# stripe/rainier

Hardware: AMD Instinct MI355X
Metric: leapfrog steps/sec (all chains) (higher is better)
Workload: dtype f64

## Files before the change

rainier_amd/csrc/engine.cpp:

```cpp
#include <hip/hip_runtime.h>
#include <hip/hiprtc.h>

#include <cmath>
#include <chrono>
#include <cstdio>
#include <cstdlib>
#include <cstring>
#include <algorithm>
#include <atomic>
#include <fstream>
#include <functional>
#include <map>
#include <memory>
#include <mutex>
#include <string>
#include <thread>
#include <vector>

#include <dlfcn.h>
#include <sys/stat.h>
#include <unistd.h>

#include "../../include/rainier_hip.h"
#include "../../include/rainier_hip_rir.h"
#include "device/rh_shared.h"
#include "rir.hpp"
#include "optimize.hpp"
#include "engine_internal.hpp"
#include "lanes_plan.hpp"

const char *const kSharedSrc =
#include "gen/rh_shared.inc"
    ;
const char *const kPreludeSrc =
#include "gen/rh_prelude.inc"
    ;
static const char *kEngineSrc =
#include "gen/rh_engine.inc"
    ;
namespace {
thread_local std::string g_err;
std::atomic<long> g_compiles{0};

uint64_t fnv1a(const std::string &s, uint64_t h = 1469598103934665603ULL) {
  for (unsigned char ch : s) { h ^= ch; h *= 1099511628211ULL; }
  return h;
}

std::string lib_dir() {
  Dl_info info;
  if (dladdr((void *)&fnv1a, &info) && info.dli_fname) {
    std::string p(info.dli_fname);
    auto pos = p.find_last_of('/');
// ... 71 lines not shown
  KSet variants[8];
  bool want_nuts = false;
  rh::Program prog;
  rh::EmitOptions eopt;
  rh::EmitInfo info;
  int mass_vec = 9;
  std::string source, err, arch;
  std::vector<char> code;
  int device = 0;
  bool loaded = false;
  hipModule_t module = nullptr;
  hipFunction_t k_chain = nullptr, k_density = nullptr, k_selftest = nullptr, k_grad = nullptr, k_tick = nullptr;
  hipFunction_t k_grad_fused = nullptr;
  hipFunction_t k_absorb = nullptr;
  hipFunction_t k_compact = nullptr;
  int ncols_max = 0, glm_ncols = 0;
  hipFunction_t k_grad_glm = nullptr;
  bool glm_small = false;
  bool lk_lds = false;
  bool has_glm = false;
  int n_row_targets_hint = 0;
  bool shape_guessed = false;
  bool rows_unroll_auto = true;
  bool unroll_auto = false;
  int gather_waves = 3;
  int glm_w = 4;
  int n_row_targets = 0, grad_k = 4, nacc_max = 1;
  hipFunction_t k_grad_gather = nullptr, k_density_fin = nullptr;
  hipFunction_t k_grad_gather_scan = nullptr;
  std::vector<std::vector<int>> goff_host;
// ... 48 lines not shown
  int chains = 0;
  void *d_state = nullptr, *d_seeds = nullptr, *d_mass = nullptr, *d_draws = nullptr, *d_stats = nullptr, *d_running = nullptr;
  int it_done = 0;
  bool started = false, warmed = false;
  hipEvent_t e0 = nullptr, e1 = nullptr;
  double kernel_ms = 0, total_ms = 0;
  int64_t chain_slots = 0, steady_launches = 0, steady_evals = 0;
  double steady_ms = 0;
  int64_t launches = 0;
  bool tick_engine = false;
  int nsplit = 0, xcd_aware = 1;
  bool compact = true;
  void *d_qbuf = nullptr, *d_active = nullptr;
  void *d_rec[2] = {nullptr, nullptr};
  bool fuse = false;
  std::vector<Lane> lanes;
  std::vector<rh_chain_stats_dev> last_stats;
  int64_t grads_at_reset = 0;
};
int guard(rh_model *m, const std::function<void()> &fn) {
  try { fn(); return RH_OK; }
  catch (const Fail &f) { g_err = f.msg; if (m) m->err = f.msg; return f.code; }
  catch (const std::exception &e) { g_err = e.what(); if (m) m->err = e.what(); return RH_E_INVALID; }
}
DrawsView sampler_draws(rh_sampler *s) {
  return {s->d_draws, s->m->device, s->m->stream, s->chains, s->it_done, (int)s->m->prog.n_params, s->cfg.iterations, &s->m->mu, &s->m->err, s->m};
}

namespace {

// ... 266 lines not shown
    if (bad("rh_chain_kernel") && m->eopt.chain_waves != 1 && !rh::knob("RH_CHAIN_WAVES")) { m->eopt.chain_waves = 1; again(); continue; }
    if (bad("rh_grad_kernel") || bad("rh_grad_fused_kernel")) {
      bool lighter = true;
      if (m->eopt.grad_unroll > 1) m->eopt.grad_unroll /= 2;
      else if (m->info.grad_k > 1) m->eopt.grad_chains = m->info.grad_k / 2;
      else if (m->eopt.grad_pipeline != 0) m->eopt.grad_pipeline = 0;
      else lighter = false;
      if (lighter) { again(); continue; }
    }
    if (!usable() && heavier()) { again(); continue; }
    if (marker) m->code = build_source(m->arch, m->source, extra);
    return;
  }
}

hipFunction_t fit_kernel(const std::vector<char> &code, hipModule_t module, const char *name, std::string *why = nullptr) {
  std::string w;
  const int h = kernel_health(code, name, &w);
  if (h != KH_OK) {
    if (why) *why = h == KH_BAD ? w : std::string(name) + " is not part of this build";
    return nullptr;
  }
  hipFunction_t f = nullptr;
  HIPCHK(hipModuleGetFunction(&f, module, name));
  return f;
}

void load_module(rh_model *m) {
  HIPCHK(hipSetDevice(m->device));
  HIPCHK(hipModuleLoadData(&m->module, m->code.data()));
  HIPCHK(hipModuleGetFunction(&m->k_selftest, m->module, "rh_selftest_kernel"));
// ... 130 lines not shown
  return ks;
}


int apply_compile_opts(rh_model *m, const rh_compile_opts *opts) {
  if (!opts) return -1;
  if (opts->struct_size != (int32_t)sizeof(rh_compile_opts)) throw Fail{RH_E_INVALID, "rh_compile_opts.struct_size mismatch"};
  if (opts->math_mode != RH_MATH_FAST && opts->math_mode != RH_MATH_STRICT) throw Fail{RH_E_INVALID, "unknown math_mode"};
  m->eopt.strict_math = opts->math_mode == RH_MATH_STRICT;
  m->eopt.fp_contract = opts->fp_contract != 0;
  if (opts->rows_unroll < 0 || opts->rows_unroll > 64) throw Fail{RH_E_INVALID, "rows_unroll out of range [0,64]"};
  if (opts->rows_unroll > 0) { m->eopt.rows_unroll = opts->rows_unroll; m->rows_unroll_auto = false; }
  if (opts->grad_chains < 0 || opts->grad_chains > 16 || opts->grad_unroll < 0 || opts->grad_unroll > 16)
    throw Fail{RH_E_INVALID, "grad_chains / grad_unroll out of range [0,16]"};
  m->eopt.grad_chains = opts->grad_chains; m->eopt.grad_unroll = opts->grad_unroll;
  m->eopt.factor_outputs = opts->factor_outputs != 0;
  if (opts->with_nuts < 0 || opts->with_nuts > 7) throw Fail{RH_E_INVALID, "with_nuts: unknown variant bits"};
  m->want_nuts = opts->with_nuts != 0;
  return opts->device;
}

void load_program(rh_model *m, const void *rir, size_t rir_len, const double *const *columns, const int64_t *nrows,
                  std::vector<const double *> &cols, std::vector<int64_t> &nrows_m, bool tables_without_data = false) {
  std::string err;
  if (!rh::parse_rir(rir, rir_len, m->prog, err)) throw Fail{RH_E_INVALID, err};
  if (m->prog.kind != 0) throw Fail{RH_E_INVALID, "a density program (header kind 0) is needed"};
  const uint32_t caller_cols = m->prog.n_cols_total;
  std::vector<uint32_t> old1, old2;
  bool lift = true;
  if (const char *e = rh::knob("RH_LIFT_CONSTANTS")) lift = std::atoi(e) != 0;
// ... 326 lines not shown
  const int rc = guard(m, [&] {
    int ndev = 0;
    if (hipGetDeviceCount(&ndev) != hipSuccess || ndev == 0) throw Fail{RH_E_DEVICE, "no HIP device available"};
    int dev = device;
    if (dev < 0) HIPCHK(hipGetDevice(&dev));
    if (dev >= ndev) throw Fail{RH_E_INVALID, "device ordinal out of range"};
    m->prog = src->prog; m->eopt = src->eopt; m->info = src->info; m->want_nuts = src->want_nuts;
    m->source = src->source; m->nacc_max = src->nacc_max; m->grad_k = src->grad_k; m->has_glm = src->has_glm;
    m->glm_small = src->glm_small; m->glm_w = src->glm_w; m->lk_lds = src->lk_lds; m->gather_waves = src->gather_waves;
    m->goff_host = src->goff_host; m->gather_count = src->gather_count; m->col_len = src->col_len; m->col_src = src->col_src;
    m->rows_total = src->rows_total; m->data = src->data; m->data.cols = nullptr;
    m->n_row_targets_hint = src->n_row_targets_hint; m->rows_unroll_auto = src->rows_unroll_auto; m->unroll_auto = src->unroll_auto;
    m->shape_guessed = src->shape_guessed; m->synth_cols = src->synth_cols; m->ncols_max = src->ncols_max; m->glm_ncols = src->glm_ncols;
    m->device = dev;
    m->arch = device_arch(dev);
    if (m->arch == src->arch) m->code = src->code; else build_code(m);
    load_module(m);
    if (m->want_nuts) (void)load_variant(m, 1);
    size_t c = 0;
    for (size_t t = 0; t < m->prog.targets.size(); t++) {
      const auto &T = m->prog.targets[t];
      for (uint32_t j = 0; j < T.n_cols; j++, c++) {
        const size_t bytes = (size_t)m->data.nrows[t] * sizeof(double);
        void *d = nullptr;
        HIPCHK(hipMalloc(&d, bytes ? bytes : 8));
        m->dev_cols.push_back(d);
        if (bytes) HIPCHK(hipMemcpyPeer(d, dev, src->dev_cols[c], src->device, bytes));
      }
    }
    for (size_t rt = 0; rt < src->goff_dev.size(); rt++) {
      const size_t bytes = m->goff_host[rt].size() * sizeof(int);
// ... 11 lines not shown
  *out = m;
  return RH_OK;
}

extern "C" void rh_model_destroy(rh_model *m) {
  if (!m) return;
  if (m->module || !m->dev_cols.empty()) {
    hipSetDevice(m->device);
    for (void *d : m->dev_cols) hipFree(d);
    if (m->d_coltab) hipFree(m->d_coltab);
    if (m->d_kpool) hipFree(m->d_kpool);
    for (void *d : m->goff_dev) hipFree(d);
    if (m->stream) hipStreamDestroy(m->stream);
    for (int v = 1; v < 8; v++)
      if (m->variants[v].module && m->variants[v].module != m->module) hipModuleUnload(m->variants[v].module);
    if (m->module) hipModuleUnload(m->module);
  }
  delete m;
}
extern "C" int rh_model_nvars(const rh_model *m) { return m ? (int)m->prog.n_params : -RH_E_INVALID; }
extern "C" const char *rh_model_hip_source(const rh_model *m) { return m ? m->source.c_str() : ""; }
extern "C" int rh_optimize(rh_model *m, const double *x0, int32_t starts, int32_t max_evals, double *x_out,
                           int32_t *evals_out, int32_t *status_out) {
  if (!m || !m->loaded) { g_err = "rh_optimize: model not loaded"; return RH_E_INVALID; }
  if (!x_out || starts <= 0) { m->err = g_err = "rh_optimize: bad arguments"; return RH_E_INVALID; }
  std::string err;
  int rc = rh::lbfgs_multistart((int)m->prog.n_params, starts, x0, max_evals,
                                [m](const double *q, int k, double *lp, double *gr) { return rh_density_eval(m, q, k, lp, gr); },
                                x_out, evals_out, status_out, err);
  (void)err;
// ... 70 lines not shown
extern "C" int rh_lower_report_data(const void *rir, size_t rir_len, const double *const *columns, const int64_t *nrows,
                                    const rh_compile_opts *opts, const char *arch, char **src_out, size_t *code_size, char **report) {
  rh_model m;
  const int rc = guard(nullptr, [&] {
    std::vector<int64_t> nrows_in;
    std::vector<const double *> colv;
    (void)apply_compile_opts(&m, opts);
    load_program(&m, rir, rir_len, columns, nrows, colv, nrows_in);
    bool all_cols = true;
    for (const double *c : colv) all_cols = all_cols && c != nullptr;
    if (all_cols && ((columns && nrows) || !m.synth_cols.empty())) { std::vector<int64_t> nrows_t; canonicalize(&m, colv.data(), nrows_in.data(), nrows_t); }
    assemble_source(&m);
    m.arch = arch && *arch ? arch : "gfx950";
    if (code_size) {
      build_code(&m);
      *code_size = m.code.size();
    }
    if (src_out) {
      std::string text = m.source;
      if (!m.info.kpool.empty()) {
        text += "\n// rh_kpool " + std::to_string(m.info.kpool.size()) + ":";
        char buf[40];
        for (double v : m.info.kpool) { std::snprintf(buf, sizeof buf, " %a", v); text += buf; }
        text += "\n";
      }
      *src_out = (char *)std::malloc(text.size() + 1); std::memcpy(*src_out, text.c_str(), text.size() + 1);
    }
    if (!code_size) return;
    std::vector<char> vcode;
    if (opts && opts->with_nuts) vcode = build_variant_code(&m, opts->with_nuts & 7);
    if (report) {
      std::string r = "attempts=" + std::to_string(m.compile_attempts) + " rows_unroll=" + std::to_string(m.eopt.rows_unroll) +
                      " grad_unroll=" + std::to_string(m.eopt.grad_unroll) + " grad_k=" + std::to_string(m.info.grad_k) +
                      " chain_waves=" + std::to_string(m.eopt.chain_waves) + " grad_pipeline=" + std::to_string(m.eopt.grad_pipeline) +
                      " chunk=" + std::to_string(m.eopt.chunk) + " bigu=" + std::to_string(m.eopt.big_unroll) + " gather=" + std::to_string((int)m.info.gather_mode) + " row_targets=" + std::to_string(m.n_row_targets_hint) + "\n";
      r += code_report(m.code, "base");
      if (!vcode.empty()) r += code_report(vcode, "variant" + std::to_string(opts->with_nuts & 7));
      *report = (char *)std::malloc(r.size() + 1); std::memcpy(*report, r.c_str(), r.size() + 1);
    }
  });
  return rc;
}
extern "C" int rh_lower_only(const void *rir, size_t rir_len, const rh_compile_opts *opts, const char *arch,
                             char **src_out, size_t *code_size) {
  return rh_lower_only_data(rir, rir_len, nullptr, nullptr, opts, arch, src_out, code_size);
}
extern "C" void rh_free(void *p) { std::free(p); }
extern "C" int rh_simplify_rir(const void *rir, size_t rir_len, int fast, void **out, size_t *out_len) {
  return guard(nullptr, [&] {
    rh::Program P; std::string err;
    if (!rh::parse_rir(rir, rir_len, P, err)) throw Fail{RH_E_INVALID, err};
    const std::vector<unsigned char> b = rh::write_rir(rh::simplify(P, fast != 0));
// ... 91 lines not shown
};

int default_nsplit(const rh_model *m, int chains) {
  const int ngroups = (chains + m->grad_k - 1) / m->grad_k;
  int64_t max_rows = 1;
  for (size_t t = 0; t < m->prog.targets.size(); t++) if (m->prog.targets[t].n_cols) max_rows = std::max<int64_t>(max_rows, m->data.nrows[t]);
  int nsplit = (int)std::max<int64_t>(1, ((m->eopt.grad_pipeline == 2 ? 2048 : 4096) + ngroups - 1) / ngroups);
  if (m->info.gather_mode) nsplit = (int)std::max<int64_t>(1, (16384 + ngroups - 1) / ngroups);
  if (const char *e = rh::knob("RH_GATHER_WG")) if (m->info.gather_mode) nsplit = (int)std::max<int64_t>(1, (std::atoi(e) + ngroups - 1) / ngroups);
  if (m->k_grad_glm) { const int ctiles = (chains + 15) / 16; nsplit = (int)std::max<int64_t>(1, (2048 + ctiles - 1) / ctiles); }
  nsplit = ((nsplit + 7) / 8) * 8;
  const int64_t cap = std::max<int64_t>(8, (max_rows / 2048) / 8 * 8);
  return (int)std::min<int64_t>(nsplit, cap);
}

void launch_grad(rh_model *m, GatherBufs *gb, void *d_q, void *d_list, void *d_nlive, void *d_vflag, void *d_partial, void *d_graderr, void *d_running,
                 int chains, int nsplit, int xcd, hipStream_t stream = nullptr) {
  if (!stream) stream = m->stream;
  const int ngroups = (chains + m->grad_k - 1) / m->grad_k;
  if (m->info.gather_mode) {
    void *ga[] = {&m->data, &gb->gd, &d_q, &d_list, &d_nlive, &d_vflag, &d_partial, &d_graderr, &d_running, &chains, &nsplit};
    if (gb->any_big) launch(m->k_grad_gather, (unsigned)(ngroups * nsplit), 64, stream, ga);
    if (gb->any_small) launch(m->k_grad_gather_scan, (unsigned)(ngroups * nsplit), 64, stream, ga);
    return;
  }
  void *args[] = {&m->data, &d_q, &d_list, &d_nlive, &d_vflag, &d_partial, &d_graderr, &d_running, &chains, &nsplit, &xcd};
  if (m->k_grad_glm) {
    const int ctiles = (chains + 15) / 16;
    const unsigned blocks = (unsigned)(((ctiles + m->glm_w - 1) / m->glm_w) * nsplit);
    const unsigned tile = (unsigned)m->glm_ncols * 66u * (unsigned)sizeof(double);
    const unsigned lds = (2u * tile + (m->lk_lds ? 6176u : 0u) <= 160u * 1024u ? 2u : 1u) * tile;
    HIPCHK(hipModuleLaunchKernel(m->k_grad_glm, blocks, 1, 1, 64u * m->glm_w, 1, 1, lds, stream, args, nullptr));
  } else
// ... 16 lines not shown
  if (use_tick && !m->tick_ok) { m->err = g_err = "the tick engine's kernels of this model are not fit to run: " + m->tick_why; return RH_E_UNSUPPORTED; }
  if (!use_tick && !m->density_ok) { m->err = g_err = "rh_density_kernel of this model is not fit to run: " + m->density_why; return RH_E_UNSUPPORTED; }
  std::lock_guard<std::mutex> lk(m->mu);
  int lookup_err = 0;
  const int rc = guard(m, [&] {
    HIPCHK(hipSetDevice(m->device));
    const int n = (int)m->prog.n_params;
    DevBuf bq(sizeof(double) * n * chains), bl(sizeof(double) * chains), bg(sizeof(double) * n * chains), be(sizeof(int));
    const bool bigth = m->info.bign && !m->info.gather_mode && (n > 512 || m->eopt.chunk > 0);
    DevBuf btot(bigth ? sizeof(double) * (size_t)(n + 1) * chains : 8);
    void *dq = bq.p, *dl = bl.p, *dg = bg.p, *de = be.p, *dtot = btot.p;
    HIPCHK(hipMemcpyAsync(dq, q, sizeof(double) * n * chains, hipMemcpyHostToDevice, m->stream));
    HIPCHK(hipMemsetAsync(de, 0, sizeof(int), m->stream));
    int ch = chains;
    if (use_tick) {
      int nsplit = grad_splits > 0 ? grad_splits : (m->info.gather_mode ? 64 : default_nsplit(m, chains));
      GatherBufs gb;
      if (m->info.gather_mode) gb.build(m, chains, nsplit);
      const size_t pbytes = sizeof(double) * (size_t)m->n_row_targets * nsplit * chains * m->nacc_max;
      DevBuf bpart(pbytes), brun(sizeof(int)), blist(sizeof(int) * chains);
      { std::vector<int> ident((size_t)chains);
        for (int c = 0; c < chains; c++) ident[(size_t)c] = c;
        HIPCHK(hipMemcpyAsync(blist.p, ident.data(), sizeof(int) * chains, hipMemcpyHostToDevice, m->stream));
        HIPCHK(hipStreamSynchronize(m->stream)); }
      HIPCHK(hipMemsetAsync(bpart.p, 0, pbytes, m->stream));
      int xcd = 1;
      if (const char *e = rh::knob("RH_XCD_AWARE")) xcd = std::atoi(e);
      void *dnl = nullptr;
      std::unique_ptr<DevBuf> bnl;
      if (const char *e = rh::knob("RH_EVAL_LIVE")) {
        std::vector<int> live;
        for (const char *p = e; *p;) { char *q2; long v = std::strtol(p, &q2, 10); if (q2 == p) break; if (v >= 0 && v < chains) live.push_back((int)v); p = *q2 ? q2 + 1 : q2; }
        std::sort(live.begin(), live.end());
        live.erase(std::unique(live.begin(), live.end()), live.end());
        if (!live.empty()) {
          const int nl = (int)live.size();
          HIPCHK(hipMemcpyAsync(blist.p, live.data(), sizeof(int) * nl, hipMemcpyHostToDevice, m->stream));
          bnl.reset(new DevBuf(sizeof(int)));
          HIPCHK(hipMemcpyAsync(bnl->p, &nl, sizeof(int), hipMemcpyHostToDevice, m->stream));
          HIPCHK(hipStreamSynchronize(m->stream));
          dnl = bnl->p;
        }
      }
      launch_grad(m, &gb, dq, blist.p, dnl, nullptr, bpart.p, de, brun.p, chains, nsplit, xcd);
      void *dpart = bpart.p;
      if (m->info.gather_mode) {
        void *fa[] = {&m->data, &gb.gd, &dq, &dpart, &dl, &dg, &de, &ch, &nsplit, &dtot};
        launch(m->k_density_fin, (unsigned)chains, 64, m->stream, fa);
      } else {
        void *fa[] = {&m->data, &dq, &dpart, &dl, &dg, &de, &ch, &nsplit, &dtot};
        launch(m->k_density_fin, (unsigned)chains, 64, m->stream, fa);
      }
      HIPCHK(hipMemcpyAsync(logp, dl, sizeof(double) * chains, hipMemcpyDeviceToHost, m->stream));
      HIPCHK(hipMemcpyAsync(grad, dg, sizeof(double) * n * chains, hipMemcpyDeviceToHost, m->stream));
      HIPCHK(hipMemcpyAsync(&lookup_err, de, sizeof(int), hipMemcpyDeviceToHost, m->stream));
      HIPCHK(hipStreamSynchronize(m->stream));
      return;
    }
    void *args[] = {&m->data, &dq, &dl, &dg, &de, &ch, &dtot};
// ... 168 lines not shown
      for (int c = 0; c < chains; c++) {
        const double nn = cfg->rng_next_gaussian ? cfg->rng_next_gaussian[c] : std::nan("");
        rec[2 * c] = seeds[c];
        std::memcpy(&rec[2 * c + 1], &nn, sizeof nn);
      }
      HIPCHK(hipMemcpy(s->d_seeds, rec.data(), sizeof(int64_t) * rec.size(), hipMemcpyHostToDevice));
    }
    std::vector<double> mass(n, 1.0);
    if (cfg->mass_tuner == RH_MASS_STATIC_DIAG) mass.assign(cfg->static_mass, cfg->static_mass + n);
    HIPCHK(hipMemcpy(s->d_mass, mass.data(), sizeof(double) * n, hipMemcpyHostToDevice));
    HIPCHK(hipMemset(s->d_draws, 0, draws_bytes));
    HIPCHK(hipEventCreate(&s->e0));
    HIPCHK(hipEventCreate(&s->e1));
    s->last_stats.resize(chains);
    if (s->tick_engine) {
      int nsplit = cfg->grad_splits;
      if (nsplit <= 0) nsplit = default_nsplit(m, chains);
      int subf = cfg->sampler == RH_SAMPLER_HMC ? 1 : 8;
      if (const char *e = rh::knob("RH_SUBF")) { subf = 1; while (subf * 2 <= std::atoi(e) && subf < 64) subf *= 2; }
      if (const char *e = rh::knob("RH_COMPACT")) s->compact = std::atoi(e) != 0;
      { int64_t max_rows = 1;
        for (size_t t = 0; t < m->prog.targets.size(); t++) if (m->prog.targets[t].n_cols) max_rows = std::max<int64_t>(max_rows, m->data.nrows[t]);
        while (subf > 1 && max_rows / ((int64_t)nsplit * subf) < 1024) subf >>= 1; }
      if (!m->k_compact) s->compact = false;
      nsplit *= subf;
      if (nsplit > 65536) throw Fail{RH_E_INVALID, "grad_splits too large"};
      s->nsplit = nsplit;
      if (const char *e = rh::knob("RH_XCD_AWARE")) s->xcd_aware = std::atoi(e);
      HIPCHK(hipMalloc(&s->d_qbuf, sizeof(double) * n * chains));
      HIPCHK(hipMalloc(&s->d_active, sizeof(int) * chains));
      HIPCHK(hipMemset(s->d_qbuf, 0, sizeof(double) * n * chains));
      HIPCHK(hipMemset(s->d_active, 0, sizeof(int) * chains));
      const size_t rec_u64 = (size_t)(3 * n + 8);
      {
        bool fuse = m->k_grad_fused && m->k_absorb && s->k_tick == m->k_tick && cfg->sampler == RH_SAMPLER_HMC && !m->k_grad_glm;
        if (const char *e = rh::knob("RH_FUSE")) fuse = fuse && std::atoi(e) != 0;
        if (fuse) {
          const size_t rec_bytes = sizeof(uint64_t) * rec_u64 * chains;
          for (int k = 0; k < 2; k++) { HIPCHK(hipMalloc(&s->d_rec[k], rec_bytes)); HIPCHK(hipMemset(s->d_rec[k], 0, rec_bytes)); }
          s->fuse = true;
        }
      }
      int forced = 0;
      if (const char *e = rh::knob("RH_LANES")) forced = std::atoi(e) == 1 ? 1 : (std::atoi(e) == 2 ? 2 : 0);
      const rh_plan::LaneCut cut = rh_plan::lanes_cut(chains, m->k_grad_glm ? 16 : m->grad_k, nsplit, m->k_grad_glm ? m->glm_w : 1,
                                                      device_cus(m->device), forced);
      s->lanes.resize((size_t)cut.lanes);
      const size_t iters_alloc = (size_t)cfg->iterations;
      for (int li = 0; li < cut.lanes; li++) {
        Lane &L = s->lanes[(size_t)li];
        const int f = cut.first[li], lc = cut.count[li];
        L.first = f; L.chains = lc;
        if (li == 0) L.stream = m->stream;
        else { HIPCHK(hipStreamCreateWithFlags(&L.stream, hipStreamNonBlocking)); L.own_stream = true; }
        HIPCHK(hipEventCreate(&L.e0));
        HIPCHK(hipEventCreate(&L.e1));
        L.state = (uint64_t *)s->d_state + (size_t)f * s->state_words;
        L.seeds = (int64_t *)s->d_seeds + (size_t)2 * f;
        L.draws = (double *)s->d_draws + (size_t)f * iters_alloc * n;
        L.stats = (rh_chain_stats_dev *)s->d_stats + f;
        L.qbuf = (double *)s->d_qbuf + (size_t)f * n;
// ... 64 lines not shown
                      &L.active, &partial, &L.d_graderr, &lst, &nl, &chains, &nsplit, &stop, &fresh};
      launch(s->k_tick, (unsigned)chains, 64, L.stream, args);
    } else {
      void *args[] = {&m->data, &s->cfg, &L.state, &L.seeds, &s->d_mass, &L.draws, &L.stats, &L.d_running, &L.qbuf,
                      &L.active, &partial, &L.d_graderr, &lst, &nl, &chains, &nsplit, &stop, &fresh};
      launch(s->k_tick, (unsigned)chains, 64, L.stream, args);
    }
    if (s->compact) {
      void *lg = (int *)L.d_livelog + log_slot;
      void *ca[] = {&L.active, &L.d_list, &L.d_nlive, &lg, &chains};
      launch(m->k_compact, 1u, 1024, L.stream, ca);
    }
  };
  auto grad = [&](Lane &L, void *partial) {
    launch_grad(m, L.gb, L.qbuf, L.d_list, s->compact ? L.d_nlive : nullptr ,
                value_free ? L.active : nullptr, partial, L.d_graderr, L.d_running, L.chains, nsplit, xcd, L.stream);
  };
  auto grad_fused = [&](Lane &L, void *partial_in, void *partial_out, void *rec_in, void *rec_out) {
    int chains = L.chains;
    void *live_n = s->compact ? L.d_nlive : nullptr;
    void *args[] = {&m->data, &L.qbuf, &L.d_list, &live_n, &partial_in, &partial_out, &L.d_graderr, &L.d_running, &L.state, &rec_in, &rec_out,
                    &chains, &nsplit, &xcd};
    launch(m->k_grad_fused, (unsigned)(((chains + m->grad_k - 1) / m->grad_k) * nsplit), 64, L.stream, args);
  };
  auto absorb = [&](Lane &L, void *rec) {
    int chains = L.chains;
    void *args[] = {&L.state, &rec, &L.qbuf, &L.active, &chains};
    launch(m->k_absorb, (unsigned)chains, 64, L.stream, args);
  };
  const int Ltraj = std::max(1, s->cfg.hmc_steps);
  const bool fuse_now = s->fuse && s->warmed && s->cfg.sampler == RH_SAMPLER_HMC && Ltraj > 1;
// ... 271 lines not shown
  if (warmed) *warmed = s->warmed ? 1 : 0;
  if (iterations_done) *iterations_done = s->it_done;
  return RH_OK;
}
extern "C" int rh_sampler_timing(rh_sampler *s, rh_timing *out, int reset) {
  if (!s || !out) { g_err = "rh_sampler_timing: NULL"; return RH_E_INVALID; }
  std::lock_guard<std::mutex> lk(s->m->mu);
  return guard(s->m, [&] {
    fetch_stats(s);
    int64_t grads = 0;
    for (auto &d : s->last_stats) grads += d.gradient_evaluations;
    std::memset(out, 0, sizeof(*out));
    out->kernel_ms = s->kernel_ms; out->total_ms = s->total_ms; out->launches = s->launches;
    out->density_evals = grads - s->grads_at_reset;
    out->row_chain_evals = out->density_evals * s->m->rows_total;
    std::snprintf(out->dominant_kernel, sizeof out->dominant_kernel, s->tick_engine ? (s->m->info.gather_mode ? "rh_grad_gather_kernel" : s->m->k_grad_glm ? "rh_grad_glm_kernel" : (s->fuse && s->warmed && s->cfg.hmc_steps > 1) ? "rh_grad_fused_kernel" : "rh_grad_kernel") : "rh_chain_kernel");
    out->chain_slots = s->tick_engine ? s->chain_slots : out->density_evals;
    out->steady_kernel_ms = s->steady_ms; out->steady_launches = s->steady_launches; out->steady_density_evals = s->steady_evals;
    if (reset) { s->kernel_ms = 0; s->total_ms = 0; s->launches = 0; s->grads_at_reset = grads; s->chain_slots = 0; s->steady_ms = 0; s->steady_launches = 0; s->steady_evals = 0; }
  });
}

extern "C" int rh_sample(rh_model *m, const rh_config *cfg, const int64_t *seeds, int32_t chains, double *draws,
                         double *mass_diag, rh_chain_stats *stats) {
  rh_sampler *s = nullptr;
  int rc = rh_sampler_create(m, cfg, seeds, chains, &s);
  if (rc != RH_OK) return rc;
  rc = rh_sampler_warmup(s);
  if (rc == RH_OK) rc = rh_sampler_run(s, cfg->iterations);
  if (rc == RH_OK && draws && cfg->iterations > 0) rc = rh_sampler_draws(s, 0, cfg->iterations, draws);
  if (rc == RH_OK) rc = rh_sampler_stats(s, stats, mass_diag);
  rh_sampler_destroy(s);
  return rc;
}

extern "C" int rh_sample_multi(rh_model *const *models, int32_t n_models, const rh_config *cfg, const int64_t *seeds,
                               int32_t chains, double *draws, double *mass_diag, rh_chain_stats *stats) {
  if (!models || n_models <= 0 || !cfg || !seeds || chains <= 0) { g_err = "rh_sample_multi: bad arguments"; return RH_E_INVALID; }
  if (cfg->struct_size != (int32_t)sizeof(rh_config)) { g_err = "rh_config.struct_size mismatch"; return RH_E_INVALID; }
  const int nv = models[0] ? rh_model_nvars(models[0]) : -1;
  for (int g = 0; g < n_models; g++) {
    if (!models[g] || !models[g]->loaded) { g_err = "rh_sample_multi: model " + std::to_string(g) + " not loaded"; return RH_E_INVALID; }
    if (rh_model_nvars(models[g]) != nv) { g_err = "rh_sample_multi: the models differ (nvars)"; return RH_E_INVALID; }
  }
  const int G = std::min<int>(n_models, chains);
  int splits_all = cfg->grad_splits;
  if (splits_all <= 0 && models[0]->n_row_targets > 0) splits_all = default_nsplit(models[0], chains);
  std::vector<int> first((size_t)G + 1, 0);
  for (int g = 0; g < G; g++) first[(size_t)g + 1] = first[(size_t)g] + chains / G + (g < chains % G ? 1 : 0);
  std::vector<int> rcs((size_t)G, RH_OK);
  std::vector<std::string> errs((size_t)G);
  std::vector<std::thread> th;
  for (int g = 0; g < G; g++)
    th.emplace_back([&, g] {
      const int c0 = first[(size_t)g], nc = first[(size_t)g + 1] - c0;
      rh_config c = *cfg;
      c.grad_splits = splits_all;
      if (cfg->rng_next_gaussian) c.rng_next_gaussian = cfg->rng_next_gaussian + c0;
      const size_t per_chain = (size_t)cfg->iterations * (size_t)nv;
      rcs[(size_t)g] = rh_sample(models[g], &c, seeds + c0, nc, draws ? draws + (size_t)c0 * per_chain : nullptr,
                                 mass_diag ? mass_diag + (size_t)c0 * nv : nullptr, stats ? stats + c0 : nullptr);
      if (rcs[(size_t)g] != RH_OK) errs[(size_t)g] = rh_last_error(models[g]);
    });
  for (auto &t : th) t.join();
  for (int g = 0; g < G; g++)
    if (rcs[(size_t)g] != RH_OK) { g_err = "shard " + std::to_string(g) + ": " + errs[(size_t)g]; return rcs[(size_t)g]; }
  return RH_OK;
}
```

rainier_amd/csrc/lanes_plan.hpp:

```cpp
#ifndef RH_LANES_PLAN_HPP
#define RH_LANES_PLAN_HPP

#include <algorithm>
#include <vector>

namespace rh_plan {
struct LaneCut { int lanes, first[2], count[2]; };
inline LaneCut lanes_cut(int chains, int group, int nsplit, int waves_per_wg, int cus, int forced) {
  LaneCut one = {1, {0, 0}, {chains, 0}};
  const int ngroups = (chains + group - 1) / group;
  if (forced == 1 || ngroups < 2) return one;
  const int cg = std::max(1, std::min(ngroups - 1, (chains + group) / (2 * group)));
  const int cut = cg * group;
  const long long smaller = std::min(cg, ngroups - cg);
  if (forced != 2 && smaller * nsplit * waves_per_wg < 4LL * cus) return one;
  return {2, {0, cut}, {cut, chains - cut}};
}

inline double busy_shares(int n, const double *t0, const double *t1, double *share) {
  struct End { double t; int kind, i; };
  std::vector<End> ends;
  ends.reserve((size_t)2 * n);
  for (int i = 0; i < n; i++) {
    share[i] = 0.0;
    ends.push_back({t0[i], 0, i});
    ends.push_back({std::max(t0[i], t1[i]), 1, i});
  }
  std::sort(ends.begin(), ends.end(), [](const End &a, const End &b) { return a.t != b.t ? a.t < b.t : (a.kind != b.kind ? a.kind < b.kind : a.i < b.i); });
  std::vector<int> open;
  double uni = 0.0, prev = 0.0;
  for (const End &e : ends) {
// ... 14 lines not shown
```

Before: 3.057 million.

## Add lane-walk gradient kernel with chain-per-lane row streaming for large HMC runs

Adds a separate gradient kernel in which each lane owns chains (two chains per lane) and the waves of a workgroup stream disjoint row ranges. Column values are read through the constant address space, R rows are unrolled at a time, and per-wave partial sums are reduced through shared memory. The kernel is compiled separately and only kept if it has no spills or scratch use. It is selected automatically for static HMC with many chains and many row evaluations, and comes with its own split count. Fused gradient kernels are turned off when it is selected, and the extra compile adds build time and code complexity.

```diff
diff --git a/rainier_amd/csrc/device/rh_lane.hip.h b/rainier_amd/csrc/device/rh_lane.hip.h
--- /dev/null
+++ b/rainier_amd/csrc/device/rh_lane.hip.h
@@ -0,0 +1,108 @@
+#if RH_NROWTARGETS > 0 && !RH_HAS_GATHER && !RH_BIGTH && !RH_BIGN && !RH_LK_LDS
+#ifndef RH_LANE_W
+#define RH_LANE_W 8
+#endif
+#ifndef RH_LANE_R
+#define RH_LANE_R 8
+#endif
+#ifndef RH_LANE_C
+#define RH_LANE_C 2
+#endif
+typedef const double __attribute__((address_space(4))) *rh_ccol_t;
+template <int T, bool NV>
+RH_DEV void rh_lane_targets(const double (&th)[RH_LANE_C][RH_NTH], const rh_model_data &d, const int w, const int split, const int nsplit,
+                            const int *__restrict__ lp, const int nvalid, const int chains, double *__restrict__ partial,
+                            double *red, int &err) {
+  if constexpr (T < RH_NTARGETS) {
+    typedef rh_target<T> TG;
+    if constexpr (TG::HAS_ROWS) {
+      constexpr int NC = TG::NCOLS, R = RH_LANE_R, C = RH_LANE_C, W = RH_LANE_W;
+      constexpr int NA = TG::NACC > 0 ? TG::NACC : 1;
+      const int lane = threadIdx.x & 63;
+      double inv[C][TG::NINV > 0 ? TG::NINV : 1];
+#pragma unroll
+      for (int k = 0; k < C; k++) TG::invariants(th[k], inv[k], err);
+      const long long n = d.nrows[T];
+      const long long blocks = (n + R - 1) / R, per = (blocks + nsplit - 1) / nsplit, perw = (per + W - 1) / W;
+      long long s0 = (long long)split * per * R, s1 = s0 + per * R;
+      if (s0 > n) s0 = n;
+      if (s1 > n) s1 = n;
+      long long r0 = s0 + (long long)w * perw * R, r1 = r0 + perw * R;
+      if (r0 > s1) r0 = s1;
+      if (r1 > s1) r1 = s1;
+      rh_ccol_t cp[NC];
+#pragma unroll
+      for (int j = 0; j < NC; j++) cp[j] = (rh_ccol_t)d.cols[TG::COL0 + j];
+      double acc[C][NA];
+#pragma unroll
+      for (int k = 0; k < C; k++)
+#pragma unroll
+        for (int o = 0; o < NA; o++) acc[k][o] = 0.0;
+      long long kb = r0;
+      for (; kb + R <= r1; kb += R) {
+        double c[R][NC];
+#pragma unroll
+        for (int u = 0; u < R; u++)
+#pragma unroll
+          for (int j = 0; j < NC; j++) c[u][j] = cp[j][kb + u];
+#pragma unroll
+        for (int u = 0; u < R; u++)
+#pragma unroll
+          for (int k = 0; k < C; k++) rh_row<TG, NV>(th[k], inv[k], c[u], acc[k], err);
+      }
+      for (; kb < r1; kb++) {
+        double c[NC];
+#pragma unroll
+        for (int j = 0; j < NC; j++) c[j] = cp[j][kb];
+#pragma unroll
+        for (int k = 0; k < C; k++) rh_row<TG, NV>(th[k], inv[k], c, acc[k], err);
+      }
+#pragma unroll
+      for (int k = 0; k < C; k++)
+#pragma unroll
+        for (int o = 0; o < NA; o++) red[((w * C + k) * NA + o) * 64 + lane] = acc[k][o];
+      __syncthreads();
+      for (int t = threadIdx.x; t < C * NA * 64; t += 64 * W) {
+        const int ko = t >> 6, l = t & 63, k = ko / NA, o = ko - k * NA;
+        double s = red[ko * 64 + l];
+#pragma unroll
+        for (int ww = 1; ww < W; ww++) s += red[(ww * C * NA + ko) * 64 + l];
+        const int slot = k * 64 + l;
+        if (slot < nvalid) partial[(((size_t)TG::ROWT * nsplit + split) * chains + lp[slot]) * RH_NACC_MAX + o] = s;
+      }
+      __syncthreads();
+    }
+    rh_lane_targets<T + 1, NV>(th, d, w, split, nsplit, lp, nvalid, chains, partial, red, err);
+  }
+}
+extern "C" __global__ void __launch_bounds__(64 * RH_LANE_W)
+rh_grad_lane_kernel(const rh_model_data d, const double *__restrict__ q, const int *__restrict__ list, const int *__restrict__ nlive,
+                    const int *__restrict__ vflag, double *__restrict__ partial, int *__restrict__ err_out, int *__restrict__ n_running,
+                    const int chains, const int nsplit, const int xcd_aware) {
+  __shared__ double red[RH_LANE_W * RH_LANE_C * RH_NACC_MAX * 64];
+  const int lane = threadIdx.x & 63, w = __builtin_amdgcn_readfirstlane((int)(threadIdx.x >> 6));
+  const int b = blockIdx.x;
+  if (b == 0 && threadIdx.x == 0) *n_running = 0;
+  const int nl = rh_live_count(nlive, chains);
+  int split, group;
+  rh_grad_map(b, nsplit, xcd_aware, split, group);
+  const int slot0 = group * (64 * RH_LANE_C);
+  if (slot0 >= nl) return;
+  double th[RH_LANE_C][RH_NTH];
+  bool gonly = rh_any_value_only<0>::v && vflag != nullptr;
+#pragma unroll
+  for (int k = 0; k < RH_LANE_C; k++) {
+    const int c = rh_live_chain(list, slot0 + k * 64 + lane, nl);
+    if constexpr (rh_any_value_only<0>::v) gonly = gonly && vflag[c] == 2;
+#pragma unroll
+    for (int i = 0; i < RH_NVARS; i++) th[k][i] = q[(size_t)c * RH_NVARS + i];
+  }
+  int err = 0;
+  if constexpr (rh_any_value_only<0>::v) {
+    if (__all(gonly)) rh_lane_targets<0, false>(th, d, w, split, nsplit, list + slot0, nl - slot0, chains, partial, red, err);
+    else rh_lane_targets<0, true>(th, d, w, split, nsplit, list + slot0, nl - slot0, chains, partial, red, err);
+  } else
+  rh_lane_targets<0, true>(th, d, w, split, nsplit, list + slot0, nl - slot0, chains, partial, red, err);
+  if (__any(err != 0) && lane == 0) atomicOr(err_out, 1);
+}
+#endif
diff --git a/rainier_amd/csrc/engine.cpp b/rainier_amd/csrc/engine.cpp
--- a/rainier_amd/csrc/engine.cpp
+++ b/rainier_amd/csrc/engine.cpp
@@ -13,6 +13,7 @@
 #include <map>
 #include <memory>
 #include <mutex>
+#include <sstream>
 #include <string>
 #include <thread>
 #include <vector>
@@ -37,6 +38,9 @@
     ;
 static const char *kEngineSrc =
 #include "gen/rh_engine.inc"
+    ;
+static const char *kLaneSrc =
+#include "gen/rh_lane.inc"
     ;
 namespace {
 thread_local std::string g_err;
@@ -138,6 +142,11 @@
   hipFunction_t k_grad_fused = nullptr;
   hipFunction_t k_absorb = nullptr;
   hipFunction_t k_compact = nullptr;
+  std::vector<char> lane_code;
+  hipModule_t lane_module = nullptr;
+  hipFunction_t k_grad_lane = nullptr;
+  int grad_chains_req = 0;
+  bool lane_tried = false;
   int ncols_max = 0, glm_ncols = 0;
   hipFunction_t k_grad_glm = nullptr;
   bool glm_small = false;
@@ -216,6 +225,7 @@
   void *d_qbuf = nullptr, *d_active = nullptr;
   void *d_rec[2] = {nullptr, nullptr};
   bool fuse = false;
+  bool lane_walk = false;
   std::vector<Lane> lanes;
   std::vector<rh_chain_stats_dev> last_stats;
   int64_t grads_at_reset = 0;
@@ -512,7 +522,64 @@
   }
 }
 
-hipFunction_t fit_kernel(const std::vector<char> &code, hipModule_t module, const char *name, std::string *why = nullptr) {
+int lane_ncols_max(const rh_model *m) {
+  int ncols_max = 0;
+  for (const auto &T : m->prog.targets) ncols_max = std::max<int>(ncols_max, (int)T.n_cols);
+  return ncols_max;
+}
+bool lane_eligible(const rh_model *m) {
+  const int ncols_max = lane_ncols_max(m);
+  const bool glm = m->has_glm && m->n_row_targets_hint == 1 && !m->glm_small;
+  return m->n_row_targets_hint > 0 && !m->info.gather_mode && !m->info.bign && m->eopt.chunk == 0 && !glm && !m->lk_lds &&
+         m->grad_chains_req == 0 && !m->want_nuts && rh_plan::lane_walk_fits_r(ncols_max, m->nacc_max, 4);
+}
+void build_lane_code(rh_model *m) {
+  m->lane_code.clear();
+  m->lane_tried = true;
+  if (!lane_eligible(m)) return;
+  const char *e = rh::knob("RH_HIPRTC_EXTRA");
+  const std::string extra = e ? e : "";
+  const bool cache = !std::getenv("RH_NO_KERNEL_CACHE");
+  for (int R : {8, 4}) {
+    if (!rh_plan::lane_walk_fits_r(lane_ncols_max(m), m->nacc_max, R)) continue;
+    const std::string src = (R == rh_plan::kLaneR ? std::string() : "#define RH_LANE_R " + std::to_string(R) + "\n") + m->source + "\n" + kLaneSrc;
+    const std::string marker = cache_path(m->arch, src, extra) + ".lane.unfit";
+    std::vector<char> mk;
+    if (cache && read_file(marker, mk) && std::string(mk.begin(), mk.end()).compare(0, marker_header().size(), marker_header()) == 0) continue;
+    bool fit = false;
+    std::string why;
+    rh::KernelMeta km;
+    std::vector<char> code;
+    try {
+      code = build_source(m->arch, src, extra, ".lane.co");
+      fit = kernel_health(code, "rh_grad_lane_kernel", &why) == KH_OK && rh::kernel_meta(code, "rh_grad_lane_kernel", km) && km.vgpr_spills == 0 &&
+            km.sgpr_spills == 0 && km.scratch_bytes == 0 && rh::kernel_touches_scratch(code, "rh_grad_lane_kernel") == 0;
+    } catch (const Fail &f) { why = f.msg; }
+    if (rh::knob("RH_BUILD_LOG"))
+      std::fprintf(stderr, "[rh build] lane walk R %d: vgprs %ld sgprs %ld spills %ld/%ld scratch %ld: %s %s\n", R, km.vgprs, km.sgprs, km.vgpr_spills,
+                   km.sgpr_spills, km.scratch_bytes, fit ? "fit" : "unfit", why.c_str());
+    if (fit) { m->lane_code = code; return; }
+    if (cache) {
+      std::remove((cache_path(m->arch, src, extra) + ".lane.co").c_str());
+      const std::string text = marker_header() + "\nrh_grad_lane_kernel\n";
+      write_file(marker, std::vector<char>(text.begin(), text.end()));
+    }
+  }
+}
+hipFunction_t fit_kernel(const std::vector<char> &code, hipModule_t module, const char *name, std::string *why = nullptr);
+hipFunction_t ensure_lane(rh_model *m) {
+  std::lock_guard<std::recursive_mutex> lk(m->engine_mu);
+  if (m->k_grad_lane) return m->k_grad_lane;
+  if (!m->k_grad || !m->k_tick || m->info.gather_mode) return nullptr;
+  if (!m->lane_tried) build_lane_code(m);
+  if (m->lane_code.empty() || m->lane_module) return nullptr;
+  HIPCHK(hipSetDevice(m->device));
+  HIPCHK(hipModuleLoadData(&m->lane_module, m->lane_code.data()));
+  m->k_grad_lane = fit_kernel(m->lane_code, m->lane_module, "rh_grad_lane_kernel", nullptr);
+  return m->k_grad_lane;
+}
+
+hipFunction_t fit_kernel(const std::vector<char> &code, hipModule_t module, const char *name, std::string *why) {
   std::string w;
   const int h = kernel_health(code, name, &w);
   if (h != KH_OK) {
@@ -673,6 +740,7 @@
   if (opts->grad_chains < 0 || opts->grad_chains > 16 || opts->grad_unroll < 0 || opts->grad_unroll > 16)
     throw Fail{RH_E_INVALID, "grad_chains / grad_unroll out of range [0,16]"};
   m->eopt.grad_chains = opts->grad_chains; m->eopt.grad_unroll = opts->grad_unroll;
+  m->grad_chains_req = opts->grad_chains;
   m->eopt.factor_outputs = opts->factor_outputs != 0;
   if (opts->with_nuts < 0 || opts->with_nuts > 7) throw Fail{RH_E_INVALID, "with_nuts: unknown variant bits"};
   m->want_nuts = opts->with_nuts != 0;
@@ -1029,7 +1097,9 @@
     m->shape_guessed = src->shape_guessed; m->synth_cols = src->synth_cols; m->ncols_max = src->ncols_max; m->glm_ncols = src->glm_ncols;
     m->device = dev;
     m->arch = device_arch(dev);
-    if (m->arch == src->arch) m->code = src->code; else build_code(m);
+    m->grad_chains_req = src->grad_chains_req;
+    if (m->arch == src->arch) { m->code = src->code; m->lane_code = src->lane_code; m->lane_tried = src->lane_tried; }
+    else build_code(m);
     load_module(m);
     if (m->want_nuts) (void)load_variant(m, 1);
     size_t c = 0;
@@ -1071,6 +1141,7 @@
     if (m->stream) hipStreamDestroy(m->stream);
     for (int v = 1; v < 8; v++)
       if (m->variants[v].module && m->variants[v].module != m->module) hipModuleUnload(m->variants[v].module);
+    if (m->lane_module) hipModuleUnload(m->lane_module);
     if (m->module) hipModuleUnload(m->module);
   }
   delete m;
@@ -1171,6 +1242,7 @@
     m.arch = arch && *arch ? arch : "gfx950";
     if (code_size) {
       build_code(&m);
+      build_lane_code(&m);
       *code_size = m.code.size();
     }
     if (src_out) {
@@ -1193,6 +1265,10 @@
                       " chunk=" + std::to_string(m.eopt.chunk) + " bigu=" + std::to_string(m.eopt.big_unroll) + " gather=" + std::to_string((int)m.info.gather_mode) + " row_targets=" + std::to_string(m.n_row_targets_hint) + "\n";
       r += code_report(m.code, "base");
       if (!vcode.empty()) r += code_report(vcode, "variant" + std::to_string(opts->with_nuts & 7));
+      if (!m.lane_code.empty()) {
+        std::istringstream all(code_report(m.lane_code, "lane"));
+        for (std::string ln; std::getline(all, ln);) if (ln.find("rh_grad_lane_kernel") != std::string::npos) r += ln + "\n";
+      }
       *report = (char *)std::malloc(r.size() + 1); std::memcpy(*report, r.c_str(), r.size() + 1);
     }
   });
@@ -1314,9 +1390,33 @@
   return (int)std::min<int64_t>(nsplit, cap);
 }
 
+int64_t lane_max_rows(const rh_model *m) {
+  int64_t max_rows = 1;
+  for (size_t t = 0; t < m->prog.targets.size(); t++) if (m->prog.targets[t].n_cols) max_rows = std::max<int64_t>(max_rows, m->data.nrows[t]);
+  return max_rows;
+}
+thread_local int g_total_chains = 0;
+thread_local int g_shard_walk = -1;
+bool walk_is_lane(rh_model *m, bool static_hmc, int total_chains) {
+  if (g_shard_walk >= 0) return g_shard_walk == 1 && ensure_lane(m) != nullptr;
+  int forced = 0;
+  if (const char *e = rh::knob("RH_GRAD_WALK")) forced = std::strcmp(e, "tile") == 0 ? 1 : (std::strcmp(e, "lane") == 0 ? 2 : 0);
+  if (!rh_plan::walk_is_lane(true, static_hmc, m->grad_chains_req, total_chains, lane_max_rows(m), forced)) return false;
+  return ensure_lane(m) != nullptr;
+}
+int lane_nsplit(const rh_model *m, int total_chains) {
+  return rh_plan::lane_nsplit(total_chains, lane_max_rows(m));
+}
+
 void launch_grad(rh_model *m, GatherBufs *gb, void *d_q, void *d_list, void *d_nlive, void *d_vflag, void *d_partial, void *d_graderr, void *d_running,
-                 int chains, int nsplit, int xcd, hipStream_t stream = nullptr) {
+                 int chains, int nsplit, int xcd, hipStream_t stream = nullptr, bool lane_walk = false) {
   if (!stream) stream = m->stream;
+  if (lane_walk) {
+    void *la[] = {&m->data, &d_q, &d_list, &d_nlive, &d_vflag, &d_partial, &d_graderr, &d_running, &chains, &nsplit, &xcd};
+    const int lgroups = (chains + rh_plan::kLaneGroup - 1) / rh_plan::kLaneGroup;
+    launch(m->k_grad_lane, (unsigned)(lgroups * nsplit), 64 * rh_plan::kLaneW, stream, la);
+    return;
+  }
   const int ngroups = (chains + m->grad_k - 1) / m->grad_k;
   if (m->info.gather_mode) {
     void *ga[] = {&m->data, &gb->gd, &d_q, &d_list, &d_nlive, &d_vflag, &d_partial, &d_graderr, &d_running, &chains, &nsplit};
@@ -1363,7 +1463,8 @@
     HIPCHK(hipMemsetAsync(de, 0, sizeof(int), m->stream));
     int ch = chains;
     if (use_tick) {
-      int nsplit = grad_splits > 0 ? grad_splits : (m->info.gather_mode ? 64 : default_nsplit(m, chains));
+      const bool lane_walk = walk_is_lane(m, false, chains);
+      int nsplit = grad_splits > 0 ? grad_splits : (m->info.gather_mode ? 64 : lane_walk ? lane_nsplit(m, chains) : default_nsplit(m, chains));
       GatherBufs gb;
       if (m->info.gather_mode) gb.build(m, chains, nsplit);
       const size_t pbytes = sizeof(double) * (size_t)m->n_row_targets * nsplit * chains * m->nacc_max;
@@ -1391,7 +1492,7 @@
           dnl = bnl->p;
         }
       }
-      launch_grad(m, &gb, dq, blist.p, dnl, nullptr, bpart.p, de, brun.p, chains, nsplit, xcd);
+      launch_grad(m, &gb, dq, blist.p, dnl, nullptr, bpart.p, de, brun.p, chains, nsplit, xcd, nullptr, lane_walk);
       void *dpart = bpart.p;
       if (m->info.gather_mode) {
         void *fa[] = {&m->data, &gb.gd, &dq, &dpart, &dl, &dg, &de, &ch, &nsplit, &dtot};
@@ -1590,8 +1691,9 @@
     HIPCHK(hipEventCreate(&s->e1));
     s->last_stats.resize(chains);
     if (s->tick_engine) {
+      s->lane_walk = walk_is_lane(m, cfg->sampler == RH_SAMPLER_HMC, g_total_chains > 0 ? g_total_chains : chains);
       int nsplit = cfg->grad_splits;
-      if (nsplit <= 0) nsplit = default_nsplit(m, chains);
+      if (nsplit <= 0) nsplit = s->lane_walk ? lane_nsplit(m, g_total_chains > 0 ? g_total_chains : chains) : default_nsplit(m, chains);
       int subf = cfg->sampler == RH_SAMPLER_HMC ? 1 : 8;
       if (const char *e = rh::knob("RH_SUBF")) { subf = 1; while (subf * 2 <= std::atoi(e) && subf < 64) subf *= 2; }
       if (const char *e = rh::knob("RH_COMPACT")) s->compact = std::atoi(e) != 0;
@@ -1609,7 +1711,7 @@
       HIPCHK(hipMemset(s->d_active, 0, sizeof(int) * chains));
       const size_t rec_u64 = (size_t)(3 * n + 8);
       {
-        bool fuse = m->k_grad_fused && m->k_absorb && s->k_tick == m->k_tick && cfg->sampler == RH_SAMPLER_HMC && !m->k_grad_glm;
+        bool fuse = m->k_grad_fused && m->k_absorb && s->k_tick == m->k_tick && cfg->sampler == RH_SAMPLER_HMC && !m->k_grad_glm && !s->lane_walk;
         if (const char *e = rh::knob("RH_FUSE")) fuse = fuse && std::atoi(e) != 0;
         if (fuse) {
           const size_t rec_bytes = sizeof(uint64_t) * rec_u64 * chains;
@@ -1619,8 +1721,8 @@
       }
       int forced = 0;
       if (const char *e = rh::knob("RH_LANES")) forced = std::atoi(e) == 1 ? 1 : (std::atoi(e) == 2 ? 2 : 0);
-      const rh_plan::LaneCut cut = rh_plan::lanes_cut(chains, m->k_grad_glm ? 16 : m->grad_k, nsplit, m->k_grad_glm ? m->glm_w : 1,
-                                                      device_cus(m->device), forced);
+      const rh_plan::LaneCut cut = rh_plan::lanes_cut(chains, s->lane_walk ? rh_plan::kLaneGroup : m->k_grad_glm ? 16 : m->grad_k, nsplit,
+                                                      s->lane_walk ? rh_plan::kLaneW : m->k_grad_glm ? m->glm_w : 1, device_cus(m->device), forced);
       s->lanes.resize((size_t)cut.lanes);
       const size_t iters_alloc = (size_t)cfg->iterations;
       for (int li = 0; li < cut.lanes; li++) {
@@ -1715,7 +1817,7 @@
   };
   auto grad = [&](Lane &L, void *partial) {
     launch_grad(m, L.gb, L.qbuf, L.d_list, s->compact ? L.d_nlive : nullptr ,
-                value_free ? L.active : nullptr, partial, L.d_graderr, L.d_running, L.chains, nsplit, xcd, L.stream);
+                value_free ? L.active : nullptr, partial, L.d_graderr, L.d_running, L.chains, nsplit, xcd, L.stream, s->lane_walk);
   };
   auto grad_fused = [&](Lane &L, void *partial_in, void *partial_out, void *rec_in, void *rec_out) {
     int chains = L.chains;
@@ -2017,7 +2119,7 @@
     out->kernel_ms = s->kernel_ms; out->total_ms = s->total_ms; out->launches = s->launches;
     out->density_evals = grads - s->grads_at_reset;
     out->row_chain_evals = out->density_evals * s->m->rows_total;
-    std::snprintf(out->dominant_kernel, sizeof out->dominant_kernel, s->tick_engine ? (s->m->info.gather_mode ? "rh_grad_gather_kernel" : s->m->k_grad_glm ? "rh_grad_glm_kernel" : (s->fuse && s->warmed && s->cfg.hmc_steps > 1) ? "rh_grad_fused_kernel" : "rh_grad_kernel") : "rh_chain_kernel");
+    std::snprintf(out->dominant_kernel, sizeof out->dominant_kernel, s->tick_engine ? (s->m->info.gather_mode ? "rh_grad_gather_kernel" : s->m->k_grad_glm ? "rh_grad_glm_kernel" : s->lane_walk ? "rh_grad_lane_kernel" : (s->fuse && s->warmed && s->cfg.hmc_steps > 1) ? "rh_grad_fused_kernel" : "rh_grad_kernel") : "rh_chain_kernel");
     out->chain_slots = s->tick_engine ? s->chain_slots : out->density_evals;
     out->steady_kernel_ms = s->steady_ms; out->steady_launches = s->steady_launches; out->steady_density_evals = s->steady_evals;
     if (reset) { s->kernel_ms = 0; s->total_ms = 0; s->launches = 0; s->grads_at_reset = grads; s->chain_slots = 0; s->steady_ms = 0; s->steady_launches = 0; s->steady_evals = 0; }
@@ -2048,7 +2150,9 @@
   }
   const int G = std::min<int>(n_models, chains);
   int splits_all = cfg->grad_splits;
-  if (splits_all <= 0 && models[0]->n_row_targets > 0) splits_all = default_nsplit(models[0], chains);
+  bool lane_all = models[0]->n_row_targets > 0;
+  for (int g = 0; g < G && lane_all; g++) lane_all = walk_is_lane(models[g], cfg->sampler == RH_SAMPLER_HMC, chains);
+  if (splits_all <= 0 && models[0]->n_row_targets > 0) splits_all = lane_all ? lane_nsplit(models[0], chains) : default_nsplit(models[0], chains);
   std::vector<int> first((size_t)G + 1, 0);
   for (int g = 0; g < G; g++) first[(size_t)g + 1] = first[(size_t)g] + chains / G + (g < chains % G ? 1 : 0);
   std::vector<int> rcs((size_t)G, RH_OK);
@@ -2061,8 +2165,10 @@
       c.grad_splits = splits_all;
       if (cfg->rng_next_gaussian) c.rng_next_gaussian = cfg->rng_next_gaussian + c0;
       const size_t per_chain = (size_t)cfg->iterations * (size_t)nv;
+      g_total_chains = chains; g_shard_walk = lane_all ? 1 : 0;
       rcs[(size_t)g] = rh_sample(models[g], &c, seeds + c0, nc, draws ? draws + (size_t)c0 * per_chain : nullptr,
                                  mass_diag ? mass_diag + (size_t)c0 * nv : nullptr, stats ? stats + c0 : nullptr);
+      g_total_chains = 0; g_shard_walk = -1;
       if (rcs[(size_t)g] != RH_OK) errs[(size_t)g] = rh_last_error(models[g]);
     });
   for (auto &t : th) t.join();
diff --git a/rainier_amd/csrc/lanes_plan.hpp b/rainier_amd/csrc/lanes_plan.hpp
--- a/rainier_amd/csrc/lanes_plan.hpp
+++ b/rainier_amd/csrc/lanes_plan.hpp
@@ -15,6 +15,26 @@
   const long long smaller = std::min(cg, ngroups - cg);
   if (forced != 2 && smaller * nsplit * waves_per_wg < 4LL * cus) return one;
   return {2, {0, cut}, {cut, chains - cut}};
+}
+
+constexpr int kLaneW = 8, kLaneR = 8, kLaneC = 2, kLaneGroup = 64 * kLaneC;
+constexpr int kLaneMinChains = 512;
+constexpr long long kLaneMinEvals = 512LL * 1000000LL;
+inline bool lane_walk_fits_r(int ncols_max, int nacc_max, int r) {
+  return ncols_max >= 1 && ncols_max * r * 2 <= 64 && nacc_max >= 1 && (long long)kLaneW * kLaneC * nacc_max * 64 * 8 <= 64 * 1024;
+}
+inline bool lane_walk_fits(int ncols_max, int nacc_max) { return lane_walk_fits_r(ncols_max, nacc_max, kLaneR); }
+inline bool walk_is_lane(bool model_has_lane, bool static_hmc, int grad_chains, int total_chains, long long max_rows, int forced) {
+  if (!model_has_lane || forced == 1) return false;
+  if (forced == 2) return true;
+  return static_hmc && grad_chains == 0 && total_chains >= kLaneMinChains && (long long)total_chains * max_rows >= kLaneMinEvals;
+}
+inline int lane_nsplit(int total_chains, long long max_rows) {
+  const long long ngroups = std::max(1, (total_chains + kLaneGroup - 1) / kLaneGroup);
+  long long nsplit = std::max<long long>(1, (8192 + ngroups * kLaneW - 1) / (ngroups * kLaneW));
+  nsplit = ((nsplit + 7) / 8) * 8;
+  const long long cap = std::max<long long>(8, (max_rows / 512) / 8 * 8);
+  return (int)std::min(nsplit, cap);
 }
 
 inline double busy_shares(int n, const double *t0, const double *t1, double *share) {
```

New measurement: 3.558 million (median of 6 runs). 1.16x the previous value.
